# f90/Wave-U-Net

Measured on AMD Instinct MI355X. Metric: waveform samples/sec fwd+bwd, M1 12-level Wave-U-Net @1/2/4/8 GPU, higher is better.
Workload: dtype f32

## Files before the change

include/wun.h:

```cpp
#ifndef WUN_H
#define WUN_H

#include <stdint.h>

#ifdef __cplusplus
extern "C" {
#endif

typedef enum wun_status {
    WUN_OK = 0,
    WUN_ERR_INVALID = -1,
    WUN_ERR_UNSUPPORTED = -2,
    WUN_ERR_HIP = -3,
    WUN_ERR_NOMEM = -4
} wun_status;

typedef struct wun_config {
    int32_t num_layers;
    int32_t num_initial_filters;
    int32_t filter_size;
    int32_t merge_filter_size;
    int32_t input_filter_size;
    int32_t output_filter_size;
    int32_t upsampling;
// ... 453 lines not shown
#define WUN_OP_INTERP_GRAD       2
#define WUN_OP_HEAD_FORWARD      3
#define WUN_OP_HEAD_DFEAT        4
#define WUN_OP_CONV_EPILOGUE     5
#define WUN_OP_BTC_TO_NCW        6
#define WUN_PATH_NONE          0
#define WUN_PATH_SCALAR        1
#define WUN_PATH_VEC4          2
#define WUN_PATH_VEC8_BF16     3
#define WUN_PATH_ONE_STAGE     4
#define WUN_PATH_TWO_STAGE     5
#define WUN_PATH_GENERIC       6
#define WUN_PATH_FOUR_POSITION 7
#define WUN_PATH_NOT_FUSED     8
#define WUN_PATH_FUSED         9
int wun_op_last_path(int op);

int64_t wun_op_conv1d_bf16_scratch(int cin, int cout, int k);
int wun_op_conv1d_bf16(const float* x, const float* w, const float* bias, float* y, float* scratch,
                       int batch, int cin, int cout, int k, int t_in, int t_out, int stride, int pad_left,
                       int lrelu, void* stream);

int64_t wun_op_conv1d_dgrad_bf16_scratch(int cin, int cout, int k);
int wun_op_conv1d_dgrad_bf16(const float* dz, const float* w, float* dx, float* scratch, int batch, int cin,
                             int cout, int k, int t_in, int t_out, int stride, int pad_left, void* stream);

int wun_op_mfma_bf16_probe(const float* a, const float* b, float* d, void* stream);

int wun_op_mfma_probe(const float* a, const float* b, float* d, void* stream);

// ... 13 lines not shown
```

wave-u-net_amd/_lib.py:

```python
import ctypes as C
import os

_HERE = os.path.dirname(os.path.abspath(__file__))
LIB_PATH = os.path.join(_HERE, os.environ.get("WUN_LIB", "libwun.so"))


class WunConfig(C.Structure):
    _fields_ = [(n, C.c_int32) for n in (
        "num_layers", "num_initial_filters", "filter_size", "merge_filter_size",
        "input_filter_size", "output_filter_size", "upsampling", "output_type", "context",
        "num_sources", "num_channels", "output_activation", "compute_dtype", "exclusive_streams")]


class WunPlanInfo(C.Structure):
    _fields_ = [("batch", C.c_int64), ("input_frames", C.c_int64), ("output_frames", C.c_int64),
                ("num_params", C.c_int64), ("arena_floats", C.c_int64),
                ("workspace_floats", C.c_int64), ("num_tensors", C.c_int64),
                ("num_outputs", C.c_int64), ("fwd_flops", C.c_double), ("bwd_flops", C.c_double),
                ("fwd_flops_dense", C.c_double), ("fwd_flops_unique", C.c_double),
                ("bwd_flops_unique", C.c_double), ("compute_dtype_effective", C.c_int64)]


class WunActivationInfo(C.Structure):
    _fields_ = [(n, C.c_int64) for n in ("offset", "batch_stride", "pitch", "channels", "frames", "t0", "tstep", "elem_bytes")]
# ... 38 lines not shown


class WunBlendWindow(C.Structure):
    _fields_ = [("pos", C.c_int64), ("row", C.c_int32), ("flags", C.c_int32)]


class WunOpHeadDesc(C.Structure):
    _fields_ = [(n, C.c_int32) for n in (
        "C", "F", "S", "difference", "Ko", "padl", "Tfeat", "Tout", "B", "tanh", "training", "feat_bf16",
        "mix_pitch", "feat_pitch", "dpre_pitch", "mix_off_feat", "mix_off_diff")]


(OP_UPSAMPLE, OP_UPSAMPLE_BACKWARD, OP_INTERP_GRAD, OP_HEAD_FORWARD, OP_HEAD_DFEAT, OP_CONV_EPILOGUE, OP_BTC_TO_NCW) = range(7)
(PATH_NONE, PATH_SCALAR, PATH_VEC4, PATH_VEC8_BF16, PATH_ONE_STAGE, PATH_TWO_STAGE, PATH_GENERIC, PATH_FOUR_POSITION,
 PATH_NOT_FUSED, PATH_FUSED) = range(10)

BLEND_NO_RISE, BLEND_NO_FALL = 1, 2
SNIPPET_SWAP, SNIPPET_NEGATE = 1, 2
SPEED_RATES, SPEED_MAX_RATIO = 8, 64
STRETCH_JOBS = 64
SNIPPET_ROWS = 24

SPEC_TT_Z, SPEC_TT_MEAN, SPEC_TT_VAR, SPEC_TT_ACT, SPEC_TT_DROPOUT = range(5)

_P = C.c_void_p
_SIGS = {
    "wun_get_padding": (C.c_int, [C.POINTER(WunConfig), C.c_int64, C.POINTER(C.c_int64),
                                  C.POINTER(C.c_int64)]),
    "wun_plan_create": (C.c_int, [C.POINTER(WunConfig), C.c_int64, C.c_int64, C.POINTER(_P)]),
    "wun_plan_destroy": (None, [_P]),
# ... 282 lines not shown
```

wave-u-net_amd/csrc/wun_backward.hip:

```cpp
#include "wun_plan_impl.h"

#include <algorithm>
#include <cstring>
#include <string>
#include <vector>

struct BucketSignal {
    const int64_t* starts; void* const* events; int n; int next;
    int ready(long long floor, hipStream_t st) {
        while (next < n && starts[next] >= floor) {
            hipError_t e = hipEventRecord((hipEvent_t)events[next], st);
            if (e != hipSuccess) return fail(WUN_ERR_HIP, std::string("hipEventRecord(bucket): ") + hipGetErrorString(e));
            ++next;
        }
        return WUN_OK;
    }
};

static int check_buckets(const int64_t* bucket_starts, void* const* bucket_events, int32_t nbuckets) {
    if (nbuckets < 0 || (nbuckets > 0 && (!bucket_starts || !bucket_events))) return fail(WUN_ERR_INVALID, "bad bucket arguments");
    for (int k = 1; k < nbuckets; ++k)
        if (bucket_starts[k] >= bucket_starts[k - 1]) return fail(WUN_ERR_INVALID, "bucket_starts must be strictly descending");
    return WUN_OK;
}
// ... 164 lines not shown
    return a;
}

int BackwardPass::tconv2(bool live, int i, bool odd, bool acc, int acc_lo, unsigned acc_len, hipStream_t st, float* part,
                         long long cap) {
    const DownShape& d = p->dsh[i];
    const ConvLayer& cl = p->down[i];
    const Buf& src = odd ? p->dz_odd[i] : p->dz_dec[i];
    const int n_in = odd ? d.n_odd : d.t_dec;
    const int out_off = odd ? d.t_odd0 : 0;
    const int out_len = odd ? 2 * (d.n_odd - 1) + Kd : d.t_in;
    ConvArgs f = conv_base(p);
    set_src0(f, ws, src, 0, d.cout);
    f.Tin = n_in; f.KW = cl.J0; f.kw_full = Kd; f.shift = cl.J0 - 1; f.W = ws + cl.wt_ph2;
    f.N = f.N0 = d.cin; f.Tout = (out_len + 1) / 2; f.Tlim = out_len; f.flags = F_PHASE2;
    set_dst0(f, ws, p->dz_dec[i - 1], out_off, &p->dec[i - 1]);
    if (acc) { f.flags |= F_ACCUM; f.acc_lo = acc_lo; f.acc_len = acc_len; }
    if (odd && cl.wt_ph2s >= 0 && !p->sw.no_odd_align) {
        const int base = d.t_odd0 - 1, extra = (base & 3) ? 2 : 0;
        if (base - extra >= 0) {
            f.KW = cl.J0s; f.shift = cl.J0s - 1 + (extra ? 1 : 0); f.W = ws + cl.wt_ph2s;
            const int len2 = out_len + 1 + extra;
            f.Tout = (len2 + 1) / 2; f.Tlim = len2;
            set_dst0(f, ws, p->dz_dec[i - 1], base - extra, &p->dec[i - 1]);
        }
    }
    const int odd_min = p->sw.odd_fuse_min;
    const int tmin = odd ? std::min(256, odd_min) : 256, wmin = odd ? odd_min : 256;
    if ((d.cin & 3) == 0 && (p->bf16 || (f.Tout >= tmin && conv_natural_wgs_phase2(f) >= wmin))) {
        HIP_TRY(dispatch(live, f, part, cap, st));
        return WUN_OK;
    }
    for (int ph = 0; ph < 2; ++ph) {
        ConvArgs a = conv_base(p);
        set_src0(a, ws, src, 0, d.cout);
        a.Tin = n_in; a.KW = cl.Jp[ph]; a.shift = cl.Jp[ph] - 1; a.W = ws + cl.wt_ph[ph];
// ... 404 lines not shown
```

wave-u-net_amd/csrc/wun_internal.h:

```cpp
#pragma once
#include <hip/hip_runtime.h>
#include <stdint.h>
#include <string>

namespace wun {

enum { LOADER_DIRECT = 0, LOADER_DEINT = 1 };

enum WunEarlyWindow { EW_DEFAULT, EW_OFF, EW_DEEP, EW_ALL };
enum WunEventScope { EV_DEFAULT, EV_SYSTEM, EV_DEVICE };
enum WunSidePrio { PRIO_DEFAULT, PRIO_LOW, PRIO_HIGH, PRIO_NORMAL };
struct WunSwitches {
    bool no_dedup = false;
    WunEarlyWindow early_window = EW_DEFAULT;
    bool odd_fuse_set = false;
    int odd_fuse_min = 64;
    bool no_odd_align = false;
    bool no_fuse_ups = false;
    bool bf16_head_serial = false;
    bool single_stream = false;
    WunSidePrio side_prio = PRIO_DEFAULT;
    WunEventScope event_scope = EV_DEFAULT;
    bool no_win = false;
    bool no_narrow = false;
    bool no_narrow_down0 = false;
    bool no_narrow_stream = false;
    int narrow_splits = 0;
    bool no_dma = false;
    bool no_k3 = false;
    int win_tk = 64;
    int bf16_lds_cap = 80;
    int tune_rounds = 4;
    bool tune_log = false;
    std::string tune_alts;
    int tune_alts_max = 6;
    float tune_alts_tol = 1.15f;
    bool dump_layout = false;
    bool profile_detail = false;
    bool win_occ = false;
};
WunSwitches wun_switches_from_env();

enum { F_LRELU = 1, F_ACCUM = 2, F_VEC4 = 4, F_PHASE2 = 8 };

struct ConvArgs {
    const float* src0; const float* src1;
    long long bs0, bs1;
    int pitch0, pitch1;
    int off0, off1;
    int C0, C1;
    int Tin;
    int shift;
    const float* W;
    const float* bias;
// ... 4 lines not shown
    long long obs0, obs1;
    int opitch0, opitch1;
    int ooff0, ooff1;
    const float* msk0; const float* msk1;
    int ostride;
    int Tout;
    float* dec; long long decbs; int decpitch;
    int dec_exp; int dec_lo; unsigned dec_len;
    float* dec1; long long dec1bs; int dec1pitch;
    int dec_off, dec1_off;
    int flags;
    int B;
    int loader;
    int Tlim;
    int kw_full;
    int force_variant;
    int force_ksplit;
    int cps;
    float* part;
    int wb_c8p, wb_npad;
    int acc_lo; unsigned acc_len;
    float* ups_y; long long ups_bs; int ups_pitch; int ups_tup; const float* ups_w;
    float* ubw_dz; const float* ubw_x; long long ubw_bs; int ubw_pitch; int ubw_n;
    int xbf, obf;
};
#define WUN_FIRST_RETIRED_VARIANT 42
#define WUN_NUM_RETIRED_VARIANTS 14
int conv_last_fused_ups();
static inline bool aligned16(const void* p) { return (reinterpret_cast<uintptr_t>(p) & 15) == 0; }
void conv_output_setup(ConvArgs& a);

struct WgradArgs {
    const float* src0; const float* src1;
    long long bs0, bs1;
    int pitch0, pitch1;
    int off0, off1;
    int C0, C1;
    int Tin;
    int shift;
    int KW;
    int loader;
    const float* dz; long long dzbs; int dzpitch; int N; int Tq;
    float* out;
// ... 91 lines not shown
};

struct PackDesc {
    long long src_off;
    long long dst_off;
    int KW, C, N, C8p, Npad;
    int src_in_ws;
};

struct WtDesc {
    long long src_off;
    long long dst_off;
    int J, C, N, k_last, k_step;
    int mode;
};

size_t conv_lds_bytes(const ConvArgs& a, int variant, const WunSwitches& sw);
int  conv_pick_variant(const ConvArgs& a);
hipError_t launch_conv(const ConvArgs& a, float* part, long long part_cap, hipStream_t s, const WunSwitches& sw);
double conv_flops(const ConvArgs& a);
long long conv_natural_wgs_phase2(const ConvArgs& a);
int conv_list_candidates(const ConvArgs& a, long long part_cap, ConvChoice* out, int maxn, const WunSwitches& sw);
bool conv_choice_ok(const ConvArgs& a, long long part_cap, int variant, int ksplit, const WunSwitches& sw);
int conv_num_variants();
int wgrad_max_units(const WgradArgs& a, const WunSwitches& sw);

int  wgrad_pick_nsplit(const WgradArgs& a, const WunSwitches& sw);
hipError_t launch_wgrad(const WgradArgs& a, hipStream_t s, const WunSwitches& sw);
void wgrad_resolved_geom(const WgradArgs& a, int& mtw, int& nw);
long long wgrad_partial_floats(const WgradArgs& a, const WunSwitches& sw);
// ... 82 lines not shown
```

wave-u-net_amd/csrc/wun_kernels.hip:

```cpp
#include "wun_device.h"

#include <cstdio>
#include <cstdlib>
#include <map>
#include <mutex>
#include <string>
#include <algorithm>
#include <vector>

namespace wun {

__device__ __forceinline__ f32x4 mfma16(float a, float b, f32x4 c) {
    return __builtin_amdgcn_mfma_f32_16x16x4f32(a, b, c, 0, 0, 0);
}

__host__ __device__ static inline int fit_pitch(int width, int mod32) {
    return width + (((mod32 - (width % 32)) % 32) + 32) % 32;
}

struct ProfSlot { std::string name; std::string tag; double flops; double bytes; hipEvent_t e0, e1, c0, c1; };
static std::vector<ProfSlot> g_prof;
static bool g_prof_on = false;
static bool g_prof_detail = false;
static std::mutex g_prof_mu;
// ... 123 lines not shown
            const int pos0 = 2 * q - a.dec_lo;
#pragma unroll
            for (int r = 0; r < 4; ++r)
                if ((unsigned)(pos0 + 2 * r) < a.dec_len) row[pos0 + 2 * r] = v[r];
        } else {
            row[q >> 1] = v[0];
            row[(q >> 1) + 1] = v[2];
        }
    }
    if (a.dec1 != nullptr) {
        float* row = a.dec1 + (long long)b * a.dec1bs + (long long)n * a.dec1pitch + a.dec1_off;
        row[q >> 1] = v[1];
        row[(q >> 1) + 1] = v[3];
    }
}
template <int MT, int NW, int WT, int WN, int CK, bool VECW, bool FOLD = false, bool XVEC = false, int KG = 1>
__global__ __launch_bounds__(256 * KG) void conv_mfma_kernel(ConvArgs a, int nTT, int nNT, int J,
                                                             int XP, int WP) {
    extern __shared__ __attribute__((aligned(16))) float lds_all[];
    const int kg = KG > 1 ? __builtin_amdgcn_readfirstlane((int)(threadIdx.x >> 8)) : 0;
    constexpr int TT = WT * MT * 16;
    constexpr int NT = WN * NW * 16;
    constexpr int NT4 = NT / 4;
    constexpr int CH = CK / 2;
    constexpr int TPR = 256 / CK;
    constexpr int XIT_D = FOLD ? (WUN_FOLD_XCAP(TT) + TPR - 1) / TPR : (TT + WUN_JMAX - 1 + TPR - 1) / TPR;
    constexpr int TPC = 256 / CH;
    constexpr int XIT_I = FOLD ? (2 * WUN_FOLD_XCAP(TT) + TPC - 1) / TPC
                               : (2 * (TT + (WUN_JMAX + 1) / 2 - 1) + TPC - 1) / TPC;
    constexpr int XIT = XVEC ? 1 : (XIT_D > XIT_I ? XIT_D : XIT_I);
    constexpr int WIT = XVEC ? 1 : (WUN_JMAX * CK * NT4 + 255) / 256;
// ... 222 lines not shown

    constexpr int KS = CK / 4;
    int arow[MT];
#pragma unroll
    for (int m = 0; m < MT; ++m) {
        arow[m] = 0;
        if constexpr (FOLD) {
            const int row = q0 + wt0 + m * 16 + li;
            int g = fast_div(row, a.Tout, inv_tout);
            const int q = row - g * a.Tout;
            g -= b;
            arow[m] = g < fold_nb ? g * fold_seg + q : 0;
        }
    }
    const bool skip_last_odd = deint && CK == 8 && (a.KW & 1);
    auto run_taps = [&](int bufoff, int j_begin, int j_end, int dlt) {
        if (j_end <= j_begin) return;
        const float* xa = Xs + bufoff + lg * XP + (FOLD ? 0 : wt0 + li) + j_begin + (deint ? (dlt >> 1) : dlt);
        const int x2off = 4 * XP + (deint ? (dlt & 1) : 0);
        (void)x2off;
        const float* wb = Ws + bufoff + (j_begin * CK + lg) * WP + wn0 + li;
        const int wstep = CK * WP;
        float a0[MT], b0[NW], a1[MT], b1[NW];
        auto ldop = [&](const float* x, const float* w, float (&av)[MT], float (&bv)[NW]) {
#pragma unroll
            for (int m = 0; m < MT; ++m) av[m] = FOLD ? x[arow[m]] : x[m * 16];
#pragma unroll
            for (int n = 0; n < NW; ++n) bv[n] = w[n * 16];
        };
        auto mm_first = [&](const float (&av)[MT], const float (&bv)[NW]) {
            acc[0][0] = mfma16(av[0], bv[0], acc[0][0]);
        };
        auto mm_rest = [&](const float (&av)[MT], const float (&bv)[NW]) {
#pragma unroll
            for (int m = 0; m < MT; ++m)
#pragma unroll
                for (int n = 0; n < NW; ++n)
                    if (m + n > 0) acc[m][n] = mfma16(av[m], bv[n], acc[m][n]);
        };
        auto pin = [&]() {
            __builtin_amdgcn_sched_group_barrier(0x008, 1, 0);
            __builtin_amdgcn_sched_group_barrier(0x100, MT + NW, 0);
            __builtin_amdgcn_sched_group_barrier(0x008, MT * NW - 1, 0);
        };
        ldop(xa, wb, a0, b0);
        if constexpr (KS == 2) {
            const int j_full = (skip_last_odd && j_end == J) ? j_end - 1 : j_end;
            for (int j = j_begin; j < j_full; ++j) {
                const bool more = j + 1 < j_end;
                mm_first(a0, b0);
                ldop(xa + x2off, wb + 4 * WP, a1, b1);
                mm_rest(a0, b0);
                pin();
                xa += more ? 1 : 0;
                wb += more ? wstep : 0;
                mm_first(a1, b1);
                ldop(xa, wb, a0, b0);
                mm_rest(a1, b1);
                pin();
            }
            if (j_full < j_end) {
                mm_first(a0, b0);
                mm_rest(a0, b0);
            }
        } else {
            const int npair = (j_end - j_begin) / 2;
            int j = j_begin;
            for (int it = 0; it < npair; ++it, j += 2) {
                const bool more2 = j + 2 < j_end;
                mm_first(a0, b0);
                ldop(xa + 1, wb + wstep, a1, b1);
                mm_rest(a0, b0);
                pin();
                xa += more2 ? 2 : 1;
                wb += more2 ? 2 * wstep : wstep;
                mm_first(a1, b1);
                ldop(xa, wb, a0, b0);
                mm_rest(a1, b1);
                pin();
            }
            if (j < j_end) {
                mm_first(a0, b0);
                mm_rest(a0, b0);
            }
        }
    };

    auto dma_chunk = [&](int chunk, int bufoff) __attribute__((always_inline)) {
        if constexpr (XVEC) {
            const int c0 = chunk * CKC;
            const bool s1 = c0 >= a.C0;
            const float* xb = s1 ? vb1 + (long long)(c0 - a.C0) * a.pitch1 : vb0 + (long long)c0 * a.pitch0;
            const int pitch = s1 ? a.pitch1 : a.pitch0, e0s = s1 ? e01 : e00;
            const int nxg = CK * XG;
#pragma unroll
            for (int i = 0; i < XDIT; ++i) {
                if (i * 256 + wave * 64 < nxg) {
                    const int pk = xdo[i];
// ... 36 lines not shown
        }
    };

    if constexpr (XVEC) {
        if (ch_lo < ch_hi) dma_chunk(ch_lo, 0);
        for (int chunk = ch_lo; chunk < ch_hi; ++chunk) {
            const int cur = ((chunk - ch_lo) & 1) * LB;
            asm volatile("s_waitcnt vmcnt(0)" ::: "memory");
            __syncthreads();
            if (chunk == ch_lo) WUN_PRIO_LO();
            if (xedge) {
                zero_fix(chunk, cur);
                __syncthreads();
            }
            if (chunk + 1 < ch_hi) dma_chunk(chunk + 1, LB - cur);
            run_taps(cur, 0, J, (chunk * CKC < a.C0) ? dl0 : dl1);
        }
    } else {
    if (ch_lo < ch_hi) load_chunk(ch_lo);
    if (ch_lo < ch_hi) store_chunk(0, ch_lo);
    __syncthreads();
    WUN_PRIO_LO();
    const int half = (J * 2) / 4;
    for (int chunk = ch_lo; chunk < ch_hi; ++chunk) {
        const int cur = ((chunk - ch_lo) & 1) * LB;
        const bool has_next = chunk + 1 < ch_hi;
        WUN_PRIO_HI();
        if (has_next) load_chunk(chunk + 1);
        WUN_PRIO_LO();
        run_taps(cur, 0, half, 0);
        WUN_PRIO_HI();
        if (has_next) store_chunk(LB - cur, chunk + 1);
        WUN_PRIO_LO();
        run_taps(cur, half, J, 0);
        __syncthreads();
    }
    }
    WUN_PRIO_HI();

    if constexpr (KG > 1) {
        __syncthreads();
        float* red = lds_all;
        if (kg > 0) {
#pragma unroll
            for (int m = 0; m < MT; ++m)
#pragma unroll
                for (int n = 0; n < NW; ++n)
                    *reinterpret_cast<f32x4*>(&red[((((kg - 1) * MT + m) * NW + n) * 256 + tid) * 4]) = acc[m][n];
        }
// ... 265 lines not shown
            }
            const int t0 = 2 * q;
            if (t0 + 7 < a.ups_tup && q + 3 < n && (a.ups_pitch & 3) == 0 && (a.ups_bs & 3) == 0) {
                *reinterpret_cast<f32x4*>(up + t0) = (f32x4){o[0], o[1], o[2], o[3]};
                *reinterpret_cast<f32x4*>(up + t0 + 4) = (f32x4){o[4], o[5], o[6], o[7]};
            } else {
#pragma unroll
                for (int r = 0; r < 8; ++r)
                    if (q + (r >> 1) < n && t0 + r < a.ups_tup) up[t0 + r] = o[r];
            }
        }
    }
}

static thread_local int t_last_fused_ups = 0;

struct ConvVariant { int MT, NW, WT, WN, CK, fold; };
static const ConvVariant kConvVariants[] = {
    {4, 2, 4, 1, 8}, {4, 3, 4, 1, 8}, {4, 4, 4, 1, 8}, {4, 5, 4, 1, 8},
    {2, 2, 4, 1, 8}, {2, 3, 4, 1, 8}, {2, 4, 4, 1, 8}, {2, 5, 4, 1, 8},
    {1, 2, 4, 1, 8}, {1, 3, 4, 1, 8},
    {1, 2, 2, 2, 8}, {1, 3, 2, 2, 8},
    {1, 2, 1, 4, 8},
    {4, 2, 4, 1, 4}, {1, 2, 4, 1, 4},
    {2, 6, 4, 1, 8}, {4, 6, 4, 1, 8},
    {3, 2, 4, 1, 8}, {3, 3, 4, 1, 8}, {3, 4, 4, 1, 8}, {3, 5, 4, 1, 8},
    {3, 6, 4, 1, 8},
    {5, 2, 4, 1, 8}, {5, 3, 4, 1, 8},
    {6, 2, 4, 1, 8}, {6, 3, 4, 1, 8},
    {4, 3, 4, 1, 4}, {2, 3, 4, 1, 4}, {3, 3, 4, 1, 4}, {2, 2, 4, 1, 4}, {3, 2, 4, 1, 4},
// ... 166 lines not shown
static hipError_t conv_launch_t(ConvArgs a, int variant, float* part, long long part_cap, hipStream_t s, const WunSwitches& sw) {
    int TT, NT, J, XP, WP;
    conv_geom(a, variant, sw, TT, NT, J, XP, WP);
    const bool phase2 = (a.flags & F_PHASE2) != 0;
    int bfac;
    const int nTT = (int)conv_mtiles(a, variant, TT, bfac);
    const int nNT = phase2 ? (a.N + NT / 2 - 1) / (NT / 2) : (a.N + NT - 1) / NT;
    size_t lds = conv_lds_bytes(a, variant, sw);
    if (KG > 1) {
        const size_t red = (size_t)(KG - 1) * MT * NW * 256 * 16;
        lds = KG * lds > red ? KG * lds : red;
        if (phase2 || lds > 160 * 1024) return hipErrorInvalidValue;
    }
    if (FOLD && !conv_fold_ok(a, variant)) return hipErrorInvalidValue;
    auto kern = conv_mfma_kernel<MT, NW, WT, WN, CK, VECW, FOLD, XVEC, KG>;
    static size_t lds_allowed = 64 * 1024;
    if (lds > lds_allowed) {
        hipError_t e = hipFuncSetAttribute((const void*)kern, hipFuncAttributeMaxDynamicSharedMemorySize, (int)lds);
        if (e != hipSuccess) return e;
        lds_allowed = lds;
    }
    const size_t lds_launch = lds;
    int ksplit, cps;
    conv_splitk(a, variant, sw, (part != nullptr && !phase2) ? part_cap : 0, ksplit, cps);
    if (a.force_ksplit > 0 && !phase2) {
        const int CKC = a.loader == LOADER_DEINT ? CK / 2 : CK;
        const int nchunks = (a.C0 + a.C1 + CKC - 1) / CKC;
        int want = a.force_ksplit > nchunks ? nchunks : a.force_ksplit;
        if (part == nullptr) want = 1;
        const long long per = (long long)a.B * a.N * ((a.Tout + 3) & ~3);
        if (want > 1 && (long long)want * per > part_cap) return hipErrorInvalidValue;
        cps = (nchunks + want - 1) / want;
        ksplit = (nchunks + cps - 1) / cps;
    }
    if (KG > 1) {
        const int CKC = a.loader == LOADER_DEINT ? CK / 2 : CK;
        const int nchunks = (a.C0 + a.C1) / CKC;
        const int want = (a.force_ksplit > 0 && part != nullptr) ? a.force_ksplit : 1;
        if ((a.C0 + a.C1) % CKC != 0 || nchunks % (KG * want) != 0) return hipErrorInvalidValue;
        const long long per = (long long)a.B * a.N * ((a.Tout + 3) & ~3);
        if (want > 1 && (long long)want * per > part_cap) return hipErrorInvalidValue;
        ksplit = want;
        cps = nchunks / (KG * want);
    }
    a.cps = cps;
    a.part = ksplit > 1 ? part : nullptr;
    const long long grid = (long long)nTT * nNT * bfac * ksplit;
    if (grid <= 0) return hipSuccess;
    char nm[64];
    snprintf(nm, sizeof(nm), "conv_mfma_kernel<%d, %d, %d, %d, %d, %s%s%s%s>", MT, NW, WT, WN, CK, VECW ? "true" : "false",
             FOLD ? ", fold" : "", XVEC ? ", dma" : "", KG > 1 ? ", k3" : "");
    {
        char tag[160];
        snprintf(tag, sizeof(tag), "C=%d N=%d T=%d K=%d ld=%d B=%d ks=%d ph2=%d acc=%d os=%d grid=%lld", a.C0 + a.C1, a.N,
                 a.Tout, a.KW, a.loader, a.B, ksplit, (a.flags & F_PHASE2) ? 1 : 0, (a.flags & F_ACCUM) ? 1 : 0,
                 a.ostride, grid);
        ProfScope ps(nm, conv_flops(a), s, tag);
        hipLaunchKernelGGL(kern, dim3((unsigned)grid), dim3(256 * KG), lds_launch, s, a, nTT, nNT, J, XP, WP);
    }
    hipError_t e = hipGetLastError();
    if (e != hipSuccess || ksplit == 1) return e;
    const long long total = (long long)a.B * a.N * (((a.Tout + 3) & ~3) >> 2);
    long long blocks = (total + 255) / 256;
    if (blocks > 4096) blocks = 4096;
    {
        const double elems = (double)a.B * a.N * a.Tout;
        double by = 4.0 * elems * (ksplit + 1 + (a.msk0 != nullptr ? 1 : 0) + ((a.flags & F_ACCUM) ? 1 : 0));
        if (a.ups_y != nullptr) by += 4.0 * (double)a.B * a.N * a.ups_tup;
        ProfScope ps("conv_splitk_epilogue_kernel", 0.0, s, "", by);
        hipLaunchKernelGGL(conv_splitk_epilogue_kernel, dim3((unsigned)blocks), dim3(256), 0, s, a, ksplit);
    }
// ... 55 lines not shown
            if (!conv_choice_ok(a, part_cap, v, ks_menu[i], sw)) {
                if (is_k3(v) && ks_menu[i] < 8) continue;
                break;
            }
            out[n].variant = v; out[n].ksplit = ks_menu[i]; ++n;
        }
    return n;
}

static_assert(sizeof(kConvVariants) / sizeof(kConvVariants[0]) == WUN_FIRST_RETIRED_VARIANT, "the retired index range follows the tile table");
static int first_k3_variant() { return WUN_FIRST_RETIRED_VARIANT + WUN_NUM_RETIRED_VARIANTS; }
int conv_num_variants() { return first_k3_variant() + kNumK3; }


int conv_last_fused_ups() { return t_last_fused_ups; }

hipError_t launch_conv(const ConvArgs& a_in, float* part, long long part_cap, hipStream_t s, const WunSwitches& sw) {
    ConvArgs a = a_in;
    t_last_fused_ups = 0;
    if (a.ups_y != nullptr && (a.dst1 != nullptr || a.msk0 != nullptr || a.ostride != 1 || a.ooff0 != 0 ||
                               (a.flags & (F_ACCUM | F_PHASE2)) != 0 || a.N0 != a.N || !aligned16(a.ups_y)))
        return hipErrorInvalidValue;
    if (a.ubw_dz != nullptr && (a.dst1 == nullptr || a.msk1 != nullptr || a.ostride != 1 || a.bias != nullptr ||
                                (a.flags & (F_ACCUM | F_PHASE2 | F_LRELU)) != 0 || a.N0 >= a.N || a.ubw_x == nullptr))
        return hipErrorInvalidValue;
    conv_output_setup(a);
    if (conv_J(a) > WUN_JMAX) return hipErrorInvalidValue;
    if (a.KW <= 0) {
        const long long total = (long long)a.B * a.N * (((a.Tout + 3) & ~3) >> 2);
        if (total <= 0) return hipSuccess;
        long long blocks = (total + 255) / 256;
        if (blocks > 4096) blocks = 4096;
        hipLaunchKernelGGL(conv_splitk_epilogue_kernel, dim3((unsigned)blocks), dim3(256), 0, s, a, 0);
        return hipGetLastError();
// ... 575 lines not shown
```

wave-u-net_amd/csrc/wun_op.hip:

```cpp
#include "wun_plan_impl.h"

#include <algorithm>
#include <cstdio>
#include <cstdlib>
#include <cstring>

namespace wun {
hipError_t launch_make_wt_one(const float* src, float* dst, WtDesc d, hipStream_t s);
}

static const long long kOpScratchFloats = 8ll << 20;
static int g_op_variant = -1, g_op_ksplit = 0;
static int g_op_wg_mtw = 0, g_op_wg_nw = 0, g_op_wg_nsplit = 0;
static int g_op_wg_bf16 = 0;
static int g_op_wg_narrow = 0;
static int g_op_wg_win = 0;
static float* g_op_copy0 = nullptr; static float* g_op_copy1 = nullptr;
static int g_op_copy_t0 = 0, g_op_copy_t1 = 0, g_op_copy_exp = 0, g_op_copy_lo = 0, g_op_copy_len = 0, g_op_acc_lo = 0, g_op_acc_len = 0;
static float* g_op_ups_y = nullptr; static const float* g_op_ups_w = nullptr;
static int g_op_ups_pitch = 0, g_op_ups_tup = 0;
static thread_local int t_op_epilogue_path = WUN_PATH_NONE;
static float* op_scratch() {
    static float* buf = nullptr;
    if (!buf && hipMalloc((void**)&buf, kOpScratchFloats * sizeof(float)) != hipSuccess) {
// ... 176 lines not shown
        a.dst0 = dx; a.obs0 = (long long)cin * t_in; a.opitch0 = t_in;
        HIP_TRY(op_launch_conv(a, s));
    } else {
        if (pad_left != 0) return fail(WUN_ERR_UNSUPPORTED, "stride-2 dgrad supports pad_left == 0 only");
        const int J0 = (k + 1) / 2;
        ConvArgs f;
        memset(&f, 0, sizeof(f));
        f.B = batch; f.ostride = 1;
        op_src(f, dz, cout, t_out);
        f.Tin = t_out; f.KW = J0; f.kw_full = k; f.shift = J0 - 1; f.W = wt_scratch; f.N = f.N0 = cin;
        f.Tout = (t_in + 1) / 2; f.Tlim = t_in; f.flags = F_PHASE2;
        f.dst0 = dx; f.obs0 = (long long)cin * t_in; f.opitch0 = t_in;
        if ((cin & 3) == 0 && conv_natural_wgs_phase2(f) >= 64) {
            WtDesc d; d.src_off = 0; d.dst_off = 0; d.J = J0; d.C = cin; d.N = cout; d.k_last = 2 * (J0 - 1);
            d.k_step = k; d.mode = 1;
            HIP_TRY(launch_make_wt_one(w, wt_scratch, d, s));
            HIP_TRY(op_launch_conv(f, s));
            return WUN_OK;
        }
        for (int ph = 0; ph < 2; ++ph) {
            const int Jp = (k - ph + 1) / 2;
            float* wt = wt_scratch + (long long)ph * k * cin * cout;
            WtDesc d; d.src_off = 0; d.dst_off = 0; d.J = Jp; d.C = cin; d.N = cout;
            d.k_last = 2 * (Jp - 1) + ph; d.k_step = 2; d.mode = 0;
            if (Jp > 0) HIP_TRY(launch_make_wt_one(w, wt, d, s));
            ConvArgs a;
            memset(&a, 0, sizeof(a));
            a.B = batch; a.ostride = 2;
            op_src(a, dz, cout, t_out);
            a.Tin = t_out; a.KW = Jp; a.shift = Jp - 1; a.W = wt; a.N = a.N0 = cin; a.Tout = (t_in - ph + 1) / 2;
// ... 212 lines not shown
    if (B < 1 || T < 1 || C < 1) return fail(WUN_ERR_INVALID, "bad shape");
    if (pitch < T) return fail(WUN_ERR_INVALID, "pitch below length");
    HIP_TRY(launch_btc_to_ncw(src, dst, B, T, C, pitch, (hipStream_t)stream));
    return WUN_OK;
}

extern "C" int wun_op_last_path(int op) {
    switch (op) {
        case WUN_OP_UPSAMPLE: return elementwise_last_path(EW_UPSAMPLE);
        case WUN_OP_UPSAMPLE_BACKWARD: return elementwise_last_path(EW_UPSAMPLE_BWD);
        case WUN_OP_INTERP_GRAD: return elementwise_last_path(EW_INTERP_GRAD);
        case WUN_OP_HEAD_FORWARD: return elementwise_last_path(EW_HEAD_FWD);
        case WUN_OP_HEAD_DFEAT: return elementwise_last_path(EW_HEAD_DFEAT);
        case WUN_OP_BTC_TO_NCW: return elementwise_last_path(EW_BTC_TO_NCW);
        case WUN_OP_CONV_EPILOGUE: return t_op_epilogue_path;
        default: return fail(WUN_ERR_INVALID, "unknown operator");
    }
}
static_assert(EW_PATH_SCALAR == WUN_PATH_SCALAR && EW_PATH_VEC4 == WUN_PATH_VEC4 && EW_PATH_VEC8_BF16 == WUN_PATH_VEC8_BF16 &&
              EW_PATH_ONE_STAGE == WUN_PATH_ONE_STAGE && EW_PATH_TWO_STAGE == WUN_PATH_TWO_STAGE &&
              EW_PATH_GENERIC == WUN_PATH_GENERIC && EW_PATH_FOUR_POSITION == WUN_PATH_FOUR_POSITION, "wun.h path values");

extern "C" int wun_op_set_conv_copies(float* copy0, int t0, int expand, int exp_lo, int exp_len, float* copy1, int t1,
                                      int acc_lo, int acc_len) {
    if ((copy0 && t0 < 1) || (copy1 && t1 < 1) || exp_len < 0 || acc_len < 0) return fail(WUN_ERR_INVALID, "bad copy geometry");
    g_op_copy0 = copy0; g_op_copy_t0 = t0; g_op_copy_exp = expand ? 1 : 0; g_op_copy_lo = exp_lo; g_op_copy_len = exp_len;
    g_op_copy1 = copy1; g_op_copy_t1 = t1; g_op_acc_lo = acc_lo; g_op_acc_len = acc_len;
    return WUN_OK;
}

extern "C" int64_t wun_op_conv1d_bf16_scratch(int cin, int cout, int k) {
    return (int64_t)k * bf16_image_groups(cin) * ((cout + 63) / 64 * 64) * 4 + 64;
}

extern "C" int wun_op_conv1d_bf16(const float* x, const float* w, const float* bias, float* y, float* scratch,
                                  int batch, int cin, int cout, int k, int t_in, int t_out, int stride, int pad_left,
// ... 47 lines not shown
    memset(&a, 0, sizeof(a));
    a.B = batch; a.ostride = 1;
    op_src(a, dz, cout, t_out);
    a.Tin = t_out; a.N = a.N0 = cin;
    a.dst0 = dx; a.obs0 = (long long)cin * t_in; a.opitch0 = t_in;
    WtDesc d; d.src_off = 0; d.dst_off = 0; d.C = cin; d.N = cout;
    PackDesc pd; pd.src_off = 0; pd.src_in_ws = 0; pd.dst_off = 0; pd.C = cout;
    if (stride == 1) {
        d.J = k; d.k_last = k - 1; d.k_step = 1; d.mode = 0;
        a.shift = k - 1 - pad_left; a.KW = k; a.Tout = t_in;
        pd.KW = k; pd.N = cin; pd.Npad = (cin + 63) / 64 * 64;
    } else {
        const int J0 = (k + 1) / 2;
        d.J = J0; d.k_last = 2 * (J0 - 1); d.k_step = k; d.mode = 1;
        a.KW = J0; a.kw_full = k; a.shift = J0 - 1; a.Tout = (t_in + 1) / 2; a.Tlim = t_in; a.flags = F_PHASE2;
        pd.KW = J0; pd.N = 2 * cin; pd.Npad = (2 * cin + 32 + 63) / 64 * 64;
    }
    pd.C8p = bf16_image_groups(cout);
    a.src0 = op_to_bf16(0, dz, (long long)batch * cout, t_out, t_out, s);
    if (!a.src0) return fail(WUN_ERR_NOMEM, "bf16 temporary");
    a.pitch0 = pad8(t_out); a.bs0 = (long long)cout * a.pitch0; a.xbf = 1; a.obf = 0;
    if (!conv_bf16_supported(a)) return fail(WUN_ERR_UNSUPPORTED, "shape not served by the bf16 kernel");
    HIP_TRY(launch_make_wt_one(w, wt, d, s));
    PackDesc* dd = nullptr;
    HIP_TRY(hipMalloc((void**)&dd, sizeof(PackDesc)));
    hipError_t e = hipMemcpyAsync(dd, &pd, sizeof(pd), hipMemcpyHostToDevice, s);
    if (e == hipSuccess) e = launch_pack_bf16(wt, img, dd, 1, (long long)pd.KW * pd.C8p * pd.Npad, s);
    a.W = img; a.wb_c8p = pd.C8p; a.wb_npad = pd.Npad;
    if (e == hipSuccess) e = launch_conv_bf16(a, s, wun_switches_from_env());
    (void)hipStreamSynchronize(s);
// ... 17 lines not shown
```

wave-u-net_amd/csrc/wun_plan.hip:

```cpp
#include "wun_plan_impl.h"

#include <cmath>
#include <cstdio>
#include <cstdlib>
#include <cstring>
#include <algorithm>
#include <string>
#include <vector>

thread_local std::string g_err;
bool g_profiling = false;

int fail(int code, const std::string& msg) {
    g_err = msg;
    return code;
}

WunSwitches wun::wun_switches_from_env() {
    WunSwitches w;
    auto set = [](const char* name) { return getenv(name) != nullptr; };
    auto num = [](const char* name, int dflt) { const char* e = getenv(name); return e ? atoi(e) : dflt; };
    w.no_dedup = set("WUN_NO_DEDUP");
    if (const char* e = getenv("WUN_EARLY_WINDOW")) w.early_window = e[0] == '0' ? EW_OFF : e[0] == 'a' ? EW_ALL : EW_DEEP;
    w.odd_fuse_set = set("WUN_ODD_FUSE_MIN");
// ... 9 lines not shown
    w.no_narrow_down0 = set("WUN_NO_NARROW_DOWN0");
    w.no_narrow_stream = num("WUN_NO_NARROW_STREAM", 0) != 0;
    if (set("WUN_NARROW_SPLITS")) w.narrow_splits = std::max(1, num("WUN_NARROW_SPLITS", 0));
    w.no_dma = set("WUN_NO_DMA");
    w.no_k3 = num("WUN_NO_K3", 0) != 0;
    { const int v = num("WUN_WIN_TK", 64); if (v == 16 || v == 32 || v == 64 || v == 128) w.win_tk = v; }
    w.bf16_lds_cap = num("WUN_BF16_LDS_CAP", 80);
    w.tune_rounds = std::max(1, num("WUN_TUNE_ROUNDS", 4));
    w.tune_log = set("WUN_TUNE_LOG");
    if (const char* e = getenv("WUN_TUNE_ALTS")) w.tune_alts = e;
    { const int v = num("WUN_TUNE_ALTS_MAX", 6); w.tune_alts_max = v > 0 ? v : 6; }
    if (const char* e = getenv("WUN_TUNE_ALTS_TOL")) { const float v = (float)atof(e); w.tune_alts_tol = v > 1.f ? v : 1.15f; }
    w.dump_layout = set("WUN_DUMP_LAYOUT");
    w.profile_detail = set("WUN_PROFILE_DETAIL");
    w.win_occ = set("WUN_WIN_OCC");
    return w;
}

static int check_config(const wun_config* c) {
    if (!c) return fail(WUN_ERR_INVALID, "config is null");
    if (c->num_layers < 1 || c->num_layers > 24) return fail(WUN_ERR_INVALID, "num_layers out of range");
    if (c->num_initial_filters < 1) return fail(WUN_ERR_INVALID, "num_initial_filters < 1");
    if (c->filter_size < 1 || c->merge_filter_size < 1 || c->output_filter_size < 1 || c->input_filter_size < 1)
        return fail(WUN_ERR_INVALID, "filter sizes must be >= 1");
    if (c->filter_size > 15 || c->merge_filter_size > 15)
        return fail(WUN_ERR_UNSUPPORTED, "filter_size / merge_filter_size > 15 not supported by the gfx950 kernels");
    if (c->upsampling != 0 && c->upsampling != 1) return fail(WUN_ERR_UNSUPPORTED, "upsampling must be linear|learned");
    if (c->output_type != 0 && c->output_type != 1) return fail(WUN_ERR_UNSUPPORTED, "output_type must be direct|difference");
    if (c->output_activation != 0 && c->output_activation != 1)
        return fail(WUN_ERR_UNSUPPORTED, "output_activation must be tanh|linear");
// ... 264 lines not shown
        p->wt.push_back(d);
        if (n > p->wt_max) p->wt_max = (int)n;
        return d.dst_off;
    };
    for (int i = 1; i < L; ++i) {
        ConvLayer& cl = p->down[i];
        cl.wt_full = add_wt(cl, cl.KW, cl.KW - 1, 1);
        if (!same) {
            for (int ph = 0; ph < 2; ++ph) {
                const int Jp = (cl.KW - ph + 1) / 2;
                cl.Jp[ph] = Jp;
                cl.wt_ph[ph] = add_wt(cl, Jp, 2 * (Jp - 1) + ph, 2);
            }
            cl.J0 = (cl.KW + 1) / 2;
            cl.wt_ph2 = add_wt2(cl, cl.J0);
            if (p->dedup) {
                cl.J0s = (cl.KW + 2) / 2;
                cl.wt_ph2s = add_wt2(cl, cl.J0s);
                p->wt.back().k_last = 2 * (cl.J0s - 1) - 1;
            }
        }
    }
    p->bott.wt_full = add_wt(p->bott, Kd, Kd - 1, 1);
    for (int j = 0; j < L; ++j) p->up[j].wt_full = add_wt(p->up[j], Ku, Ku - 1, 1);

    if (p->bf16) {
        auto add_img = [&](int in_ws, long long src_off, int K, int Cc, int Nn, int slack = 0) {
            if (Cc < 8 || K < 1) return;
            PackDesc d;
            d.src_off = src_off; d.src_in_ws = in_ws; d.KW = K; d.C = Cc; d.N = Nn;
            d.C8p = bf16_image_groups(Cc); d.Npad = (Nn + slack + 63) / 64 * 64;
            const long long items = (long long)K * d.C8p * d.Npad;
            d.dst_off = bump(w, items * 4);
            p->pack.push_back(d);
// ... 181 lines not shown
```

wave-u-net_amd/csrc/wun_plan_impl.h:

```cpp
#pragma once
#include "../../include/wun.h"
#include "wun_internal.h"

#include <cstring>
#include <map>
#include <string>
#include <vector>

using namespace wun;

struct Buf { long long off = -1; int C = 0; int T = 0; int pitch = 0; long long bs = 0; int eb = 4; };
struct ConvLayer { long long woff = 0, boff = 0; int KW = 0, Cin = 0, Cout = 0;
                   long long wt_full = -1, wt_ph[2] = {-1, -1}, wt_ph2 = -1; int Jp[2] = {0, 0}; int J0 = 0;
                   long long wt_ph2s = -1; int J0s = 0; };
struct DownShape { int cin, cout, t_in, t_conv, t_dec, tc, cs, t_ev0, n_even, t_odd0, n_odd; };
struct UpShape { int c_skip, c_cur, cout, t_cur, t_up, t_conv, crop_start; };

struct wun_plan {
    wun_config cfg;
    WunSwitches sw;
    WunEarlyWindow early_window = EW_DEEP;
    bool fuse_ups = false;
    int B = 0, Tin = 0, Tout = 0;
    int L = 0, C = 0, S = 0, Sh = 0;
    bool same = false;
    std::vector<wun_tensor_info> tensors;
    long long arena = 0, ws = 0;
    std::vector<DownShape> dsh;
    std::vector<UpShape> ush;
// ... 113 lines not shown
```

Baseline: 32.91 million.

## Skip structurally zero weight slab in phase-2 transposed conv MFMA kernel

Phase-2 (polyphase) transposed convolution weight images contain one tap/phase slab that is entirely zero because the kernel index falls outside the filter. The plan now records which slab is absent, and the MFMA conv kernel gets a templated peeled form (ZS=1 for first tap, phase 1; ZS=2 for last tap, phase 0) that skips the MFMAs and weight loads for that half-tile. This removes wasted matrix work in the backward dgrad convolutions, at the cost of extra kernel instantiations and more complex scheduling. A WUN_PHASE2_ALL_TAPS switch and a form-reporting query are added for testing.

```diff
diff --git a/include/wun.h b/include/wun.h
--- a/include/wun.h
+++ b/include/wun.h
@@ -491,6 +491,10 @@
 #define WUN_PATH_FOUR_POSITION 7
 #define WUN_PATH_NOT_FUSED     8
 #define WUN_PATH_FUSED         9
+#define WUN_OP_CONV_FORM         7
+#define WUN_CONV_FORM_PHASE2      0x100
+#define WUN_CONV_FORM_DMA         0x200
+#define WUN_CONV_FORM_TAP_SKIPPED 0x400
 int wun_op_last_path(int op);
 
 int64_t wun_op_conv1d_bf16_scratch(int cin, int cout, int k);
diff --git a/wave-u-net_amd/_lib.py b/wave-u-net_amd/_lib.py
--- a/wave-u-net_amd/_lib.py
+++ b/wave-u-net_amd/_lib.py
@@ -76,6 +76,8 @@
 (OP_UPSAMPLE, OP_UPSAMPLE_BACKWARD, OP_INTERP_GRAD, OP_HEAD_FORWARD, OP_HEAD_DFEAT, OP_CONV_EPILOGUE, OP_BTC_TO_NCW) = range(7)
 (PATH_NONE, PATH_SCALAR, PATH_VEC4, PATH_VEC8_BF16, PATH_ONE_STAGE, PATH_TWO_STAGE, PATH_GENERIC, PATH_FOUR_POSITION,
  PATH_NOT_FUSED, PATH_FUSED) = range(10)
+OP_CONV_FORM = 7
+CONV_FORM_PHASE2, CONV_FORM_DMA, CONV_FORM_TAP_SKIPPED = 0x100, 0x200, 0x400
 
 BLEND_NO_RISE, BLEND_NO_FALL = 1, 2
 SNIPPET_SWAP, SNIPPET_NEGATE = 1, 2
diff --git a/wave-u-net_amd/csrc/wun_backward.hip b/wave-u-net_amd/csrc/wun_backward.hip
--- a/wave-u-net_amd/csrc/wun_backward.hip
+++ b/wave-u-net_amd/csrc/wun_backward.hip
@@ -202,12 +202,14 @@
     set_src0(f, ws, src, 0, d.cout);
     f.Tin = n_in; f.KW = cl.J0; f.kw_full = Kd; f.shift = cl.J0 - 1; f.W = ws + cl.wt_ph2;
     f.N = f.N0 = d.cin; f.Tout = (out_len + 1) / 2; f.Tlim = out_len; f.flags = F_PHASE2;
+    f.zslab_ph = cl.zs_ph2[0]; f.zslab_j = cl.zs_ph2[1];
     set_dst0(f, ws, p->dz_dec[i - 1], out_off, &p->dec[i - 1]);
     if (acc) { f.flags |= F_ACCUM; f.acc_lo = acc_lo; f.acc_len = acc_len; }
     if (odd && cl.wt_ph2s >= 0 && !p->sw.no_odd_align) {
         const int base = d.t_odd0 - 1, extra = (base & 3) ? 2 : 0;
         if (base - extra >= 0) {
             f.KW = cl.J0s; f.shift = cl.J0s - 1 + (extra ? 1 : 0); f.W = ws + cl.wt_ph2s;
+            f.zslab_ph = cl.zs_ph2s[0]; f.zslab_j = cl.zs_ph2s[1];
             const int len2 = out_len + 1 + extra;
             f.Tout = (len2 + 1) / 2; f.Tlim = len2;
             set_dst0(f, ws, p->dz_dec[i - 1], base - extra, &p->dec[i - 1]);
diff --git a/wave-u-net_amd/csrc/wun_internal.h b/wave-u-net_amd/csrc/wun_internal.h
--- a/wave-u-net_amd/csrc/wun_internal.h
+++ b/wave-u-net_amd/csrc/wun_internal.h
@@ -38,6 +38,7 @@
     bool dump_layout = false;
     bool profile_detail = false;
     bool win_occ = false;
+    bool phase2_all_taps = false;
 };
 WunSwitches wun_switches_from_env();
 
@@ -72,6 +73,7 @@
     int loader;
     int Tlim;
     int kw_full;
+    int zslab_ph, zslab_j;
     int force_variant;
     int force_ksplit;
     int cps;
@@ -85,6 +87,8 @@
 #define WUN_FIRST_RETIRED_VARIANT 42
 #define WUN_NUM_RETIRED_VARIANTS 14
 int conv_last_fused_ups();
+enum { CONV_FORM_PHASE2 = 0x100, CONV_FORM_DMA = 0x200, CONV_FORM_TAP_SKIPPED = 0x400 };
+int conv_last_form();
 static inline bool aligned16(const void* p) { return (reinterpret_cast<uintptr_t>(p) & 15) == 0; }
 void conv_output_setup(ConvArgs& a);
 
@@ -206,6 +210,14 @@
     int J, C, N, k_last, k_step;
     int mode;
 };
+static inline void phase2_absent_slab(int J, int k_last, int k_step, int& ph, int& j) {
+    ph = j = -1;
+    for (int jj = 0; jj < J; ++jj)
+        for (int p = 0; p < 2; ++p) {
+            const int k = k_last - 2 * jj + p;
+            if (k < 0 || k >= k_step) { ph = p; j = jj; return; }
+        }
+}
 
 size_t conv_lds_bytes(const ConvArgs& a, int variant, const WunSwitches& sw);
 int  conv_pick_variant(const ConvArgs& a);
diff --git a/wave-u-net_amd/csrc/wun_kernels.hip b/wave-u-net_amd/csrc/wun_kernels.hip
--- a/wave-u-net_amd/csrc/wun_kernels.hip
+++ b/wave-u-net_amd/csrc/wun_kernels.hip
@@ -2,10 +2,12 @@
 
 #include <cstdio>
 #include <cstdlib>
+#include <cstring>
 #include <map>
 #include <mutex>
 #include <string>
 #include <algorithm>
+#include <type_traits>
 #include <vector>
 
 namespace wun {
@@ -161,7 +163,7 @@
         row[(q >> 1) + 1] = v[3];
     }
 }
-template <int MT, int NW, int WT, int WN, int CK, bool VECW, bool FOLD = false, bool XVEC = false, int KG = 1>
+template <int MT, int NW, int WT, int WN, int CK, bool VECW, bool FOLD = false, bool XVEC = false, int KG = 1, int ZS = 0>
 __global__ __launch_bounds__(256 * KG) void conv_mfma_kernel(ConvArgs a, int nTT, int nNT, int J,
                                                              int XP, int WP) {
     extern __shared__ __attribute__((aligned(16))) float lds_all[];
@@ -414,7 +416,10 @@
         }
     }
     const bool skip_last_odd = deint && CK == 8 && (a.KW & 1);
-    auto run_taps = [&](int bufoff, int j_begin, int j_end, int dlt) {
+    static_assert(ZS == 0 || (WN == 1 && CK == 8 && VECW && !FOLD && KG == 1 && ((NW % 2) == 0 || NW == 3)), "no peeled form of this tile");
+    constexpr int NW_P0 = NW == 3 ? 2 : NW / 2;
+    constexpr int NW_P1 = NW == 3 ? 1 : NW / 2;
+    auto run_taps = [&](auto first, auto last, int bufoff, int j_begin, int j_end, int dlt) __attribute__((always_inline)) {
         if (j_end <= j_begin) return;
         const float* xa = Xs + bufoff + lg * XP + (FOLD ? 0 : wt0 + li) + j_begin + (deint ? (dlt >> 1) : dlt);
         const int x2off = 4 * XP + (deint ? (dlt & 1) : 0);
@@ -422,66 +427,100 @@
         const float* wb = Ws + bufoff + (j_begin * CK + lg) * WP + wn0 + li;
         const int wstep = CK * WP;
         float a0[MT], b0[NW], a1[MT], b1[NW];
-        auto ldop = [&](const float* x, const float* w, float (&av)[MT], float (&bv)[NW]) {
+        using TileLo = std::integral_constant<int, 0>;
+        using TileHi = std::integral_constant<int, NW>;
+        auto ldop = [&](auto l0, auto l1, const float* x, const float* w, float (&av)[MT], float (&bv)[NW]) __attribute__((always_inline)) {
 #pragma unroll
             for (int m = 0; m < MT; ++m) av[m] = FOLD ? x[arow[m]] : x[m * 16];
 #pragma unroll
-            for (int n = 0; n < NW; ++n) bv[n] = w[n * 16];
+            for (int n = decltype(l0)::value; n < decltype(l1)::value; ++n) bv[n] = w[n * 16];
         };
-        auto mm_first = [&](const float (&av)[MT], const float (&bv)[NW]) {
-            acc[0][0] = mfma16(av[0], bv[0], acc[0][0]);
+        auto mm_first = [&](auto c0, const float (&av)[MT], const float (&bv)[NW]) __attribute__((always_inline)) {
+            constexpr int C0 = decltype(c0)::value;
+            acc[0][C0] = mfma16(av[0], bv[C0], acc[0][C0]);
         };
-        auto mm_rest = [&](const float (&av)[MT], const float (&bv)[NW]) {
+        auto mm_rest = [&](auto c0, auto c1, const float (&av)[MT], const float (&bv)[NW]) __attribute__((always_inline)) {
+            constexpr int C0 = decltype(c0)::value, C1 = decltype(c1)::value;
 #pragma unroll
             for (int m = 0; m < MT; ++m)
 #pragma unroll
-                for (int n = 0; n < NW; ++n)
-                    if (m + n > 0) acc[m][n] = mfma16(av[m], bv[n], acc[m][n]);
+                for (int n = C0; n < C1; ++n)
+                    if (m + n > C0) acc[m][n] = mfma16(av[m], bv[n], acc[m][n]);
         };
-        auto pin = [&]() {
+        auto kstep = [&](auto c0, auto c1, auto l0, auto l1, const float (&av)[MT], const float (&bv)[NW], const float* x,
+                         const float* w, float (&an)[MT], float (&bn)[NW]) __attribute__((always_inline)) {
+            constexpr int NC = decltype(c1)::value - decltype(c0)::value, NL = decltype(l1)::value - decltype(l0)::value;
+            mm_first(c0, av, bv);
+            ldop(l0, l1, x, w, an, bn);
+            mm_rest(c0, c1, av, bv);
             __builtin_amdgcn_sched_group_barrier(0x008, 1, 0);
-            __builtin_amdgcn_sched_group_barrier(0x100, MT + NW, 0);
-            __builtin_amdgcn_sched_group_barrier(0x008, MT * NW - 1, 0);
+            __builtin_amdgcn_sched_group_barrier(0x100, MT + NL, 0);
+            if constexpr (MT * NC > 1) __builtin_amdgcn_sched_group_barrier(0x008, MT * NC - 1, 0);
         };
-        ldop(xa, wb, a0, b0);
+        const TileLo tlo; const TileHi thi;
         if constexpr (KS == 2) {
-            const int j_full = (skip_last_odd && j_end == J) ? j_end - 1 : j_end;
-            for (int j = j_begin; j < j_full; ++j) {
-                const bool more = j + 1 < j_end;
-                mm_first(a0, b0);
-                ldop(xa + x2off, wb + 4 * WP, a1, b1);
-                mm_rest(a0, b0);
-                pin();
-                xa += more ? 1 : 0;
-                wb += more ? wstep : 0;
-                mm_first(a1, b1);
-                ldop(xa, wb, a0, b0);
-                mm_rest(a1, b1);
-                pin();
-            }
-            if (j_full < j_end) {
-                mm_first(a0, b0);
-                mm_rest(a0, b0);
+            auto full_taps = [&](int jb, int je, int jlast) __attribute__((always_inline)) {
+                for (int j = jb; j < je; ++j) {
+                    const bool more = j + 1 < jlast;
+                    kstep(tlo, thi, tlo, thi, a0, b0, xa + x2off, wb + 4 * WP, a1, b1);
+                    xa += more ? 1 : 0;
+                    wb += more ? wstep : 0;
+                    kstep(tlo, thi, tlo, thi, a1, b1, xa, wb, a0, b0);
+                }
+            };
+            constexpr bool first_p1 = ZS == 1 && decltype(first)::value;
+            constexpr bool last_p0 = ZS == 2 && decltype(last)::value;
+            if constexpr (first_p1) {
+                const std::integral_constant<int, NW_P0> p1;
+                const bool more = j_begin + 1 < j_end;
+                ldop(tlo, p1, xa, wb, a0, b0);
+                int once = 1;
+                asm volatile("" : "+s"(once));
+                for (int h = 0; h < once; ++h) {
+#pragma unroll
+                    for (int m = 0; m < MT; ++m)
+#pragma unroll
+                        for (int n = NW_P0; n < NW; ++n) asm volatile("" : "+a"(acc[m][n]));
+                    kstep(tlo, p1, tlo, p1, a0, b0, xa + x2off, wb + 4 * WP, a1, b1);
+                    xa += more ? 1 : 0;
+                    wb += more ? wstep : 0;
+                    kstep(tlo, p1, tlo, thi, a1, b1, xa, wb, a0, b0);
+                }
+                full_taps(j_begin + 1, j_end, j_end);
+            } else if constexpr (last_p0) {
+                const std::integral_constant<int, NW_P1> p0;
+                ldop(tlo, thi, xa, wb, a0, b0);
+                full_taps(j_begin, j_end - 2, j_end);
+                kstep(tlo, thi, tlo, thi, a0, b0, xa + x2off, wb + 4 * WP, a1, b1);
+                xa += 1;
+                wb += wstep;
+                kstep(tlo, thi, p0, thi, a1, b1, xa, wb, a0, b0);
+                kstep(p0, thi, p0, thi, a0, b0, xa + x2off, wb + 4 * WP, a1, b1);
+                mm_first(p0, a1, b1);
+                mm_rest(p0, thi, a1, b1);
+            } else {
+                const int j_full = (skip_last_odd && j_end == J) ? j_end - 1 : j_end;
+                ldop(tlo, thi, xa, wb, a0, b0);
+                full_taps(j_begin, j_full, j_end);
+                if (j_full < j_end) {
+                    mm_first(tlo, a0, b0);
+                    mm_rest(tlo, thi, a0, b0);
+                }
             }
         } else {
+            ldop(tlo, thi, xa, wb, a0, b0);
             const int npair = (j_end - j_begin) / 2;
             int j = j_begin;
             for (int it = 0; it < npair; ++it, j += 2) {
                 const bool more2 = j + 2 < j_end;
-                mm_first(a0, b0);
-                ldop(xa + 1, wb + wstep, a1, b1);
-                mm_rest(a0, b0);
-                pin();
+                kstep(tlo, thi, tlo, thi, a0, b0, xa + 1, wb + wstep, a1, b1);
                 xa += more2 ? 2 : 1;
                 wb += more2 ? 2 * wstep : wstep;
-                mm_first(a1, b1);
-                ldop(xa, wb, a0, b0);
-                mm_rest(a1, b1);
-                pin();
+                kstep(tlo, thi, tlo, thi, a1, b1, xa, wb, a0, b0);
             }
             if (j < j_end) {
-                mm_first(a0, b0);
-                mm_rest(a0, b0);
+                mm_first(tlo, a0, b0);
+                mm_rest(tlo, thi, a0, b0);
             }
         }
     };
@@ -548,7 +587,7 @@
                 __syncthreads();
             }
             if (chunk + 1 < ch_hi) dma_chunk(chunk + 1, LB - cur);
-            run_taps(cur, 0, J, (chunk * CKC < a.C0) ? dl0 : dl1);
+            run_taps(std::true_type(), std::true_type(), cur, 0, J, (chunk * CKC < a.C0) ? dl0 : dl1);
         }
     } else {
     if (ch_lo < ch_hi) load_chunk(ch_lo);
@@ -562,11 +601,11 @@
         WUN_PRIO_HI();
         if (has_next) load_chunk(chunk + 1);
         WUN_PRIO_LO();
-        run_taps(cur, 0, half, 0);
+        run_taps(std::true_type(), std::false_type(), cur, 0, half, 0);
         WUN_PRIO_HI();
         if (has_next) store_chunk(LB - cur, chunk + 1);
         WUN_PRIO_LO();
-        run_taps(cur, half, J, 0);
+        run_taps(std::false_type(), std::true_type(), cur, half, J, 0);
         __syncthreads();
     }
     }
@@ -862,6 +901,7 @@
 }
 
 static thread_local int t_last_fused_ups = 0;
+static thread_local int t_last_conv_form = 0;
 
 struct ConvVariant { int MT, NW, WT, WN, CK, fold; };
 static const ConvVariant kConvVariants[] = {
@@ -1058,11 +1098,16 @@
     }
     if (FOLD && !conv_fold_ok(a, variant)) return hipErrorInvalidValue;
     auto kern = conv_mfma_kernel<MT, NW, WT, WN, CK, VECW, FOLD, XVEC, KG>;
-    static size_t lds_allowed = 64 * 1024;
-    if (lds > lds_allowed) {
+    int zs = 0;
+    if constexpr (WN == 1 && CK == 8 && VECW && !FOLD && KG == 1 && ((NW % 2) == 0 || NW == 3)) {
+        if (phase2 && a.zslab_ph == 1 && a.zslab_j == 0) { zs = 1; kern = conv_mfma_kernel<MT, NW, WT, WN, CK, VECW, FOLD, XVEC, KG, 1>; }
+        if (phase2 && a.zslab_ph == 0 && a.zslab_j == J - 1 && J >= 3) { zs = 2; kern = conv_mfma_kernel<MT, NW, WT, WN, CK, VECW, FOLD, XVEC, KG, 2>; }
+    }
+    static size_t lds_allowed[3] = {64 * 1024, 64 * 1024, 64 * 1024};
+    if (lds > lds_allowed[zs]) {
         hipError_t e = hipFuncSetAttribute((const void*)kern, hipFuncAttributeMaxDynamicSharedMemorySize, (int)lds);
         if (e != hipSuccess) return e;
-        lds_allowed = lds;
+        lds_allowed[zs] = lds;
     }
     const size_t lds_launch = lds;
     int ksplit, cps;
@@ -1091,6 +1136,7 @@
     a.part = ksplit > 1 ? part : nullptr;
     const long long grid = (long long)nTT * nNT * bfac * ksplit;
     if (grid <= 0) return hipSuccess;
+    t_last_conv_form = NW | (phase2 ? CONV_FORM_PHASE2 : 0) | (XVEC ? CONV_FORM_DMA : 0) | (zs ? CONV_FORM_TAP_SKIPPED : 0);
     char nm[64];
     snprintf(nm, sizeof(nm), "conv_mfma_kernel<%d, %d, %d, %d, %d, %s%s%s%s>", MT, NW, WT, WN, CK, VECW ? "true" : "false",
              FOLD ? ", fold" : "", XVEC ? ", dma" : "", KG > 1 ? ", k3" : "");
@@ -1099,6 +1145,7 @@
         snprintf(tag, sizeof(tag), "C=%d N=%d T=%d K=%d ld=%d B=%d ks=%d ph2=%d acc=%d os=%d grid=%lld", a.C0 + a.C1, a.N,
                  a.Tout, a.KW, a.loader, a.B, ksplit, (a.flags & F_PHASE2) ? 1 : 0, (a.flags & F_ACCUM) ? 1 : 0,
                  a.ostride, grid);
+        if (phase2) snprintf(tag + strlen(tag), sizeof(tag) - strlen(tag), " zs=%d", zs);
         ProfScope ps(nm, conv_flops(a), s, tag);
         hipLaunchKernelGGL(kern, dim3((unsigned)grid), dim3(256 * KG), lds_launch, s, a, nTT, nNT, J, XP, WP);
     }
@@ -1184,10 +1231,14 @@
 
 
 int conv_last_fused_ups() { return t_last_fused_ups; }
+int conv_last_form() { return t_last_conv_form; }
 
 hipError_t launch_conv(const ConvArgs& a_in, float* part, long long part_cap, hipStream_t s, const WunSwitches& sw) {
     ConvArgs a = a_in;
     t_last_fused_ups = 0;
+    t_last_conv_form = 0;
+    if (!(a.flags & F_PHASE2) || sw.phase2_all_taps || a.zslab_ph < 0 || a.zslab_ph > 1 || a.zslab_j < 0 || a.zslab_j >= a.KW)
+        a.zslab_ph = a.zslab_j = -1;
     if (a.ups_y != nullptr && (a.dst1 != nullptr || a.msk0 != nullptr || a.ostride != 1 || a.ooff0 != 0 ||
                                (a.flags & (F_ACCUM | F_PHASE2)) != 0 || a.N0 != a.N || !aligned16(a.ups_y)))
         return hipErrorInvalidValue;
diff --git a/wave-u-net_amd/csrc/wun_op.hip b/wave-u-net_amd/csrc/wun_op.hip
--- a/wave-u-net_amd/csrc/wun_op.hip
+++ b/wave-u-net_amd/csrc/wun_op.hip
@@ -214,6 +214,7 @@
         if ((cin & 3) == 0 && conv_natural_wgs_phase2(f) >= 64) {
             WtDesc d; d.src_off = 0; d.dst_off = 0; d.J = J0; d.C = cin; d.N = cout; d.k_last = 2 * (J0 - 1);
             d.k_step = k; d.mode = 1;
+            phase2_absent_slab(d.J, d.k_last, d.k_step, f.zslab_ph, f.zslab_j);
             HIP_TRY(launch_make_wt_one(w, wt_scratch, d, s));
             HIP_TRY(op_launch_conv(f, s));
             return WUN_OK;
@@ -456,12 +457,15 @@
         case WUN_OP_HEAD_DFEAT: return elementwise_last_path(EW_HEAD_DFEAT);
         case WUN_OP_BTC_TO_NCW: return elementwise_last_path(EW_BTC_TO_NCW);
         case WUN_OP_CONV_EPILOGUE: return t_op_epilogue_path;
+        case WUN_OP_CONV_FORM: return conv_last_form();
         default: return fail(WUN_ERR_INVALID, "unknown operator");
     }
 }
 static_assert(EW_PATH_SCALAR == WUN_PATH_SCALAR && EW_PATH_VEC4 == WUN_PATH_VEC4 && EW_PATH_VEC8_BF16 == WUN_PATH_VEC8_BF16 &&
               EW_PATH_ONE_STAGE == WUN_PATH_ONE_STAGE && EW_PATH_TWO_STAGE == WUN_PATH_TWO_STAGE &&
               EW_PATH_GENERIC == WUN_PATH_GENERIC && EW_PATH_FOUR_POSITION == WUN_PATH_FOUR_POSITION, "wun.h path values");
+static_assert(CONV_FORM_PHASE2 == WUN_CONV_FORM_PHASE2 && CONV_FORM_DMA == WUN_CONV_FORM_DMA &&
+              CONV_FORM_TAP_SKIPPED == WUN_CONV_FORM_TAP_SKIPPED, "wun.h conv form bits");
 
 extern "C" int wun_op_set_conv_copies(float* copy0, int t0, int expand, int exp_lo, int exp_len, float* copy1, int t1,
                                       int acc_lo, int acc_len) {
@@ -539,6 +543,7 @@
         const int J0 = (k + 1) / 2;
         d.J = J0; d.k_last = 2 * (J0 - 1); d.k_step = k; d.mode = 1;
         a.KW = J0; a.kw_full = k; a.shift = J0 - 1; a.Tout = (t_in + 1) / 2; a.Tlim = t_in; a.flags = F_PHASE2;
+        phase2_absent_slab(d.J, d.k_last, d.k_step, a.zslab_ph, a.zslab_j);
         pd.KW = J0; pd.N = 2 * cin; pd.Npad = (2 * cin + 32 + 63) / 64 * 64;
     }
     pd.C8p = bf16_image_groups(cout);
diff --git a/wave-u-net_amd/csrc/wun_plan.hip b/wave-u-net_amd/csrc/wun_plan.hip
--- a/wave-u-net_amd/csrc/wun_plan.hip
+++ b/wave-u-net_amd/csrc/wun_plan.hip
@@ -47,6 +47,7 @@
     w.dump_layout = set("WUN_DUMP_LAYOUT");
     w.profile_detail = set("WUN_PROFILE_DETAIL");
     w.win_occ = set("WUN_WIN_OCC");
+    w.phase2_all_taps = set("WUN_PHASE2_ALL_TAPS");
     return w;
 }
 
@@ -341,10 +342,12 @@
             }
             cl.J0 = (cl.KW + 1) / 2;
             cl.wt_ph2 = add_wt2(cl, cl.J0);
+            phase2_absent_slab(p->wt.back().J, p->wt.back().k_last, p->wt.back().k_step, cl.zs_ph2[0], cl.zs_ph2[1]);
             if (p->dedup) {
                 cl.J0s = (cl.KW + 2) / 2;
                 cl.wt_ph2s = add_wt2(cl, cl.J0s);
                 p->wt.back().k_last = 2 * (cl.J0s - 1) - 1;
+                phase2_absent_slab(p->wt.back().J, p->wt.back().k_last, p->wt.back().k_step, cl.zs_ph2s[0], cl.zs_ph2s[1]);
             }
         }
     }
diff --git a/wave-u-net_amd/csrc/wun_plan_impl.h b/wave-u-net_amd/csrc/wun_plan_impl.h
--- a/wave-u-net_amd/csrc/wun_plan_impl.h
+++ b/wave-u-net_amd/csrc/wun_plan_impl.h
@@ -12,7 +12,8 @@
 struct Buf { long long off = -1; int C = 0; int T = 0; int pitch = 0; long long bs = 0; int eb = 4; };
 struct ConvLayer { long long woff = 0, boff = 0; int KW = 0, Cin = 0, Cout = 0;
                    long long wt_full = -1, wt_ph[2] = {-1, -1}, wt_ph2 = -1; int Jp[2] = {0, 0}; int J0 = 0;
-                   long long wt_ph2s = -1; int J0s = 0; };
+                   long long wt_ph2s = -1; int J0s = 0;
+                   int zs_ph2[2] = {-1, -1}, zs_ph2s[2] = {-1, -1}; };
 struct DownShape { int cin, cout, t_in, t_conv, t_dec, tc, cs, t_ev0, n_even, t_odd0, n_odd; };
 struct UpShape { int c_skip, c_cur, cout, t_cur, t_up, t_conv, crop_start; };
 
```

Result: no change. 33.12 million (median of 6 runs) (+0.6%).
